# PriUVBio/optiland_Pr

Measured on AMD Instinct MI355X. Metric: ray-surface intersections/sec at 1M pupil rays, 10-surf double-Gauss, higher is better.
Workload: dtype f64

## Files before the change

include/optiland_host.h:

```cpp
#ifndef OPTILAND_HOST_H
#define OPTILAND_HOST_H

#include "optiland_rt.h"

#ifdef __cplusplus
extern "C" {
#endif

#define ORT_HOST_ABI_VERSION 3

int ort_host_abi_version(void);

int ort_host_trace_sequential(const ort_lens* lens, const ort_rays* rays_in,
                              ort_rays* rays_out, const ort_batch* batch,
                              const ort_options* opt, double* rec, int32_t* updates,
                              int32_t* status);

int ort_host_trace_sequential_vjp(const ort_lens* lens, const ort_rays* rays_in,
                                  const ort_batch* batch, const ort_options* opt,
                                  const ort_vjp_params* params, const ort_rays* cotangent,
                                  const double* rec_cotangent, const double* rec,
                                  double* grad, const ort_rays* grad_in);

int ort_host_trace_pupil(const ort_lens* lens, const double* px, const double* py,
                         ort_rays* rays_out, const ort_batch* batch, const ort_options* opt,
                         int32_t* updates, int32_t* status);

int ort_host_trace_pupil_vjp(const ort_lens* lens, const double* px, const double* py,
                             const ort_batch* batch, const ort_options* opt,
                             const ort_vjp_params* params, const ort_rays* cotangent,
                             double* grad);

int ort_host_rms_spot(const double* x, const double* y, int64_t n, double* stats, double* rms);
int ort_host_rms_spot_vjp(const double* x, const double* y, int64_t n, const double* stats,
                          const double* grad_out, double* gx, double* gy);

int ort_host_huygens_psf(const double* ix, const double* iy, const double* iz, int64_t n_image,
                         const double* px, const double* py, const double* pz,
                         const double* amp, const double* opd_mm, int64_t n_pupil,
                         double wavelength_mm, double rp, double* psf);

int ort_host_irradiance_bin(const double* x, const double* y, const double* power, int64_t n,
                            const double* x_edges, int64_t nx, const double* y_edges,
                            int64_t ny, int32_t mode, double pixel_area, double* out);
int ort_host_irradiance_bin_vjp(const double* x, const double* y, const double* power,
                                int64_t n, const double* x_edges, int64_t nx,
                                const double* y_edges, int64_t ny, double pixel_area,
                                const double* grad_out, double* grad_x, double* grad_y,
                                double* grad_power);

int ort_host_trace_pupil_polarized(const ort_lens* lens, const double* px, const double* py,
                                   ort_rays* rays_out, const ort_batch* batch,
                                   const ort_options* opt, double* rec, int32_t* updates,
                                   int32_t* status, const ort_polarization* pol);
int ort_host_trace_sequential_polarized(const ort_lens* lens, const ort_rays* rays_in,
                                        ort_rays* rays_out, const ort_batch* batch,
                                        const ort_options* opt, double* rec, int32_t* updates,
                                        int32_t* status, const ort_polarization* pol);

int ort_host_generate_rays(const double* px, const double* py, ort_rays* rays_out,
                           const ort_batch* batch);

void ort_host_set_threads(int32_t n);

#ifdef __cplusplus
}
#endif
#endif
```

include/optiland_rt.h:

```cpp
#ifndef OPTILAND_RT_H
#define OPTILAND_RT_H

#include <stdint.h>

#ifdef __cplusplus
extern "C" {
#endif

#define ORT_ABI_VERSION 21
#define ORT_MAX_SURFACES 64

enum ort_geometry {
  ORT_GEOM_PLANE = 0,
  ORT_GEOM_STANDARD = 1,
  ORT_GEOM_EVEN_ASPHERE = 2,
  ORT_GEOM_ODD_ASPHERE = 3,
  ORT_GEOM_ZERNIKE = 4,
  ORT_GEOM_POLYNOMIAL = 5,
  ORT_GEOM_CHEBYSHEV = 6,
  ORT_GEOM_BICONIC = 7,
  ORT_GEOM_TOROIDAL = 8,
  ORT_GEOM_FORBES_QBFS = 9,
  ORT_GEOM_FORBES_Q2D = 10,
  ORT_GEOM_GRID_SAG = 11,
  ORT_GEOM_NURBS = 12
};

enum ort_surface_flags {
  ORT_SURF_REFLECTIVE = 1u << 0,
  ORT_SURF_RADIUS_INF = 1u << 1,
  ORT_SURF_APERTURE = 1u << 2,
  ORT_SURF_RECORD = 1u << 3,
  ORT_SURF_TRANSLATE = 1u << 4,
  ORT_SURF_APERTURE_PROG = 1u << 5,
  ORT_SURF_INV_R2 = 1u << 6,
  ORT_SURF_ALPHA_ALL = 1u << 7,
  ORT_SURF_ALPHA_NONE = 1u << 8,
  ORT_SURF_SLOPE_INEXACT = 1u << 9
};

enum ort_lens_flags {
  ORT_LENS_AXIAL = 1u << 0
};

enum ort_interaction {
  ORT_IA_REFRACT_REFLECT = 0,
  ORT_IA_THIN_LENS = 1,
  ORT_IA_PHASE = 2,
  ORT_IA_DIFFRACTIVE = 3
};
enum ort_phase_kind { ORT_PHASE_CONSTANT = 0, ORT_PHASE_LINEAR = 1, ORT_PHASE_RADIAL = 2 };

enum ort_cs_kind {
  ORT_CS_TRANSLATE = 0,
  ORT_CS_ROT_X = 1,
  ORT_CS_ROT_Y = 2,
  ORT_CS_ROT_Z = 3
};

typedef struct ort_cs_op {
  int32_t kind;
  int32_t reserved;
  double p[3];
} ort_cs_op;

typedef struct ort_surface {
  double radius;
  double conic;
  double tol;
  double norm_radius;
  double ap_rmax2;
  double ap_rmin2;
  int32_t geometry;
  int32_t flags;
  int32_t max_iter;
  int32_t n_coef;
  int32_t coef_off;
  int32_t mat_pre;
  int32_t mat_post;
  int32_t cs_loc_off;
  int32_t n_cs_loc;
  int32_t cs_glob_off;
  int32_t n_cs_glob;
  int32_t rec_slot;
  double cs_t[3];
  int32_t ap_off;
  int32_t ap_len;
  int32_t interaction;
  int32_t ia_off;
  double inv_r2;
  double two_r;
  double one_plus_k;
  double r_sq;
  int32_t zm_off;
  int32_t zm_deg;
} ort_surface;

enum ort_aperture_op {
  ORT_AP_RADIAL = 1,
  ORT_AP_ELLIPSE = 2,
  ORT_AP_RECT = 3,
  ORT_AP_POLYGON = 4,
  ORT_AP_UNION = 5,
  ORT_AP_INTERSECT = 6,
  ORT_AP_DIFFERENCE = 7
};

typedef struct ort_surface_optics {
  double n_pre;
  double u;
  double alpha_pre;
  double n_post;
  double u_sq;
} ort_surface_optics;

typedef struct ort_zernike_term {
  double c;
  double norm;
  int32_t n;
  int32_t m;
  int32_t rad_off;
  int32_t n_rad;
} ort_zernike_term;

enum ort_material_kind {
  ORT_MAT_IDEAL = 0,
  ORT_MAT_FORMULA_1 = 1,
  ORT_MAT_TABULATED = 10,
  ORT_MAT_ABBE = 11
};
typedef struct ort_material {
  int32_t kind;
  int32_t n_coef;
  int32_t coef_off;
  int32_t k_len;
  int32_t k_off;
  int32_t reserved;
  double n_const;
  double k_const;
} ort_material;

typedef struct ort_lens {
  const ort_surface* surfaces;
  const ort_cs_op* cs_ops;
  const double* coef;
  const ort_zernike_term* zern;
  const double* n_tab;
  const double* alpha_tab;
  const ort_surface_optics* optics;
  int32_t n_surfaces;
  int32_t n_lambda;
  int32_t n_mat;
  int32_t final_mat;
  uint32_t geometry_mask;
  uint32_t interaction_mask;
  double final_thickness;
  const ort_material* materials;
  const double* wavelengths;
  uint32_t frame_flags;
  uint32_t reserved;
} ort_lens;

typedef struct ort_rays {
  double* x;
  double* y;
  double* z;
  double* L;
  double* M;
  double* N;
  double* i;
  double* opd;
} ort_rays;

enum ort_gen_mode {
  ORT_GEN_INFINITE = 0,
  ORT_GEN_FINITE = 1,
  ORT_GEN_TELECENTRIC = 2
};
typedef struct ort_segment {
  double epd;
  double epl;
  double vx, vy;
  double x_off;
  double y_off;
  double z0;
  int32_t lambda_idx;
  int32_t mode;
} ort_segment;

enum ort_apod_kind {
  ORT_APOD_UNIFORM = 0,
  ORT_APOD_GAUSSIAN = 1,
  ORT_APOD_COSINE_SQUARED = 2,
  ORT_APOD_HANN = 3,
  ORT_APOD_POLYNOMIAL = 4,
// ... 297 lines not shown
```

optiland_pr_amd/_abi.py:

```python

from __future__ import annotations

import numpy as np

ABI_VERSION = 21
HUYGENS_CHUNK = 512
BIN_HISTOGRAM = 0
BIN_BILINEAR = 1
IRRADIANCE_TILE_PIXELS = 16384
IRRADIANCE_MAX_PIXELS = 1 << 26
VJP_UNROLLED = 0
VJP_ADJOINT = 1
AP_RADIAL = 1
AP_ELLIPSE = 2
AP_RECT = 3
AP_POLYGON = 4
AP_UNION = 5
AP_INTERSECT = 6
AP_DIFFERENCE = 7
PUPIL_UNIFORM = 0
PUPIL_HEXAPOLAR = 1
PUPIL_RANDOM = 2
PUPIL_RING = 3
PUPIL_LINE_X = 4
PUPIL_LINE_Y = 5
PUPIL_CROSS = 6
MAX_SURFACES = 64

GEOM_PLANE = 0
GEOM_STANDARD = 1
GEOM_EVEN_ASPHERE = 2
GEOM_ODD_ASPHERE = 3
GEOM_ZERNIKE = 4
GEOM_POLYNOMIAL = 5
GEOM_CHEBYSHEV = 6
GEOM_BICONIC = 7
GEOM_TOROIDAL = 8
GEOM_FORBES_QBFS = 9
GEOM_FORBES_Q2D = 10
GEOM_GRID_SAG = 11
GEOM_NURBS = 12
FREEFORM_GEOMETRIES = (GEOM_POLYNOMIAL, GEOM_CHEBYSHEV, GEOM_BICONIC, GEOM_TOROIDAL,
                       GEOM_FORBES_QBFS, GEOM_FORBES_Q2D, GEOM_GRID_SAG)
NEWTON_GEOMETRIES = (GEOM_EVEN_ASPHERE, GEOM_ODD_ASPHERE, GEOM_ZERNIKE) + FREEFORM_GEOMETRIES

SURF_REFLECTIVE = 1 << 0
SURF_RADIUS_INF = 1 << 1
SURF_APERTURE = 1 << 2
SURF_RECORD = 1 << 3
SURF_TRANSLATE = 1 << 4
SURF_APERTURE_PROG = 1 << 5
SURF_INV_R2 = 1 << 6
SURF_ALPHA_ALL = 1 << 7
SURF_ALPHA_NONE = 1 << 8
SURF_SLOPE_INEXACT = 1 << 9
LENS_AXIAL = 1 << 0

IA_REFRACT_REFLECT = 0
IA_THIN_LENS = 1
IA_PHASE = 2
IA_DIFFRACTIVE = 3
PHASE_CONSTANT = 0
PHASE_LINEAR = 1
PHASE_RADIAL = 2

CS_TRANSLATE = 0
CS_ROT_X = 1
CS_ROT_Y = 2
CS_ROT_Z = 3

GEN_INFINITE = 0
GEN_FINITE = 1
GEN_TELECENTRIC = 2

APOD_UNIFORM = 0
APOD_GAUSSIAN = 1
APOD_COSINE_SQUARED = 2
APOD_HANN = 3
APOD_POLYNOMIAL = 4
APOD_SUPER_GAUSSIAN = 5
APOD_TUKEY = 6

NEWTON_SCHEDULE = 0
NEWTON_WAVE = 1

STATUS_ZERNIKE_RANGE = 1 << 0
STATUS_CHEBYSHEV_RANGE = 1 << 1
STATUS_BAD_GEOMETRY = 1 << 2
STATUS_BAD_APODIZATION = 1 << 3

CS_OP = np.dtype(
    [("kind", "<i4"), ("reserved", "<i4"), ("p", "<f8", (3,))], align=True
)
assert CS_OP.itemsize == 32

SURFACE = np.dtype(
    [
        ("radius", "<f8"),
        ("conic", "<f8"),
        ("tol", "<f8"),
        ("norm_radius", "<f8"),
        ("ap_rmax2", "<f8"),
        ("ap_rmin2", "<f8"),
        ("geometry", "<i4"),
        ("flags", "<i4"),
        ("max_iter", "<i4"),
        ("n_coef", "<i4"),
        ("coef_off", "<i4"),
        ("mat_pre", "<i4"),
        ("mat_post", "<i4"),
        ("cs_loc_off", "<i4"),
        ("n_cs_loc", "<i4"),
        ("cs_glob_off", "<i4"),
        ("n_cs_glob", "<i4"),
        ("rec_slot", "<i4"),
        ("cs_t", "<f8", (3,)),
        ("ap_off", "<i4"),
        ("ap_len", "<i4"),
        ("interaction", "<i4"),
        ("ia_off", "<i4"),
        ("inv_r2", "<f8"),
        ("two_r", "<f8"),
        ("one_plus_k", "<f8"),
        ("r_sq", "<f8"),
        ("zm_off", "<i4"),
        ("zm_deg", "<i4"),
    ],
    align=True,
)
assert SURFACE.itemsize == 176

SURFACE_OPTICS = np.dtype(
    [("n_pre", "<f8"), ("u", "<f8"), ("alpha_pre", "<f8"), ("n_post", "<f8"), ("u_sq", "<f8")],
    align=True,
)
assert SURFACE_OPTICS.itemsize == 40

ZERNIKE_TERM = np.dtype(
    [
        ("c", "<f8"),
        ("norm", "<f8"),
        ("n", "<i4"),
        ("m", "<i4"),
        ("rad_off", "<i4"),
        ("n_rad", "<i4"),
    ],
    align=True,
)
assert ZERNIKE_TERM.itemsize == 32

SEGMENT = np.dtype(
    [
        ("epd", "<f8"),
        ("epl", "<f8"),
        ("vx", "<f8"),
        ("vy", "<f8"),
        ("x_off", "<f8"),
        ("y_off", "<f8"),
        ("z0", "<f8"),
        ("lambda_idx", "<i4"),
        ("mode", "<i4"),
    ],
    align=True,
)
assert SEGMENT.itemsize == 64

APODIZATION = np.dtype(
    [
        ("kind", "<i4"),
        ("reserved", "<i4"),
        ("p", "<f8", (4,)),
    ],
    align=True,
)
assert APODIZATION.itemsize == 40

COAT_NONE = 0
COAT_SIMPLE = 1
COAT_FRESNEL = 2
COATING = np.dtype(
    [
        ("kind", "<i4"),
        ("mat_pre", "<i4"),
        ("mat_post", "<i4"),
        ("reserved", "<i4"),
        ("transmittance", "<f8"),
        ("reflectance", "<f8"),
    ],
    align=True,
)
assert COATING.itemsize == 32
POL_IGNORE = 0
POL_MATRICES = 1
POL_POLARIZED = 2
POL_UNPOLARIZED = 3

MAT_IDEAL = 0
MAT_TABULATED = 10
MAT_ABBE = 11

MATERIAL = np.dtype(
    [
        ("kind", "<i4"),
        ("n_coef", "<i4"),
        ("coef_off", "<i4"),
        ("k_len", "<i4"),
        ("k_off", "<i4"),
        ("reserved", "<i4"),
        ("n_const", "<f8"),
# ... 30 lines not shown
```

optiland_pr_amd/csrc/ort_args.h:

```cpp
#pragma once

#include "ort_core.h"
#include "ort_interact.h"
#include "ort_material.h"
#include "ort_polar.h"

namespace ortk {

#if defined(__HIP_DEVICE_COMPILE__)
#define ORT_CONST_AS __attribute__((address_space(4)))
#else
#define ORT_CONST_AS
#endif
template <class T>
using cptr = const ORT_CONST_AS T*;
template <class T>
ORT_INLINE cptr<T> cst(const T* p) {
  return (cptr<T>)(p);
}
using PD = cptr<double>;
using PZ = cptr<ort_zernike_term>;
constexpr ort::ZSeed kNoSeed{nullptr, 0};

enum : uint32_t {
  F_KM = 15u | ort::KM_NURBS,
  F_GEN = 1u << 4,
  F_REC = 1u << 5,
  F_MONO = 1u << 6,
  F_WRAY = 1u << 7,
  F_IA = 1u << 8,
  F_AXIAL = 1u << 9,
  F_TAPE = 1u << 10,
  F_SPOT = 1u << 11,
  F_RMS = 1u << 12,
  F_STRIDE = 1u << 13,
  F_POL = 1u << 14,
};
constexpr uint32_t kAllKinds =
    ort::KM_EVEN | ort::KM_ODD | ort::KM_ZERN | ort::KM_FREE | ort::KM_NURBS;

constexpr int kTapeRows = 11;
constexpr int kHist = 4;

ORT_INLINE int tape_rows(const ort_surface& s) {
  return (s.geometry == ORT_GEOM_PLANE || s.geometry == ORT_GEOM_STANDARD) ? 7 : kTapeRows;
}
ORT_INLINE int64_t tape_row0(const ort_surface* surf, int si) {
  int64_t r = 0;
  for (int k = 0; k < si; ++k) r += tape_rows(cst(surf)[k]);
  return r;
}

struct KArgs {
  const ort_surface* surf;
  const ort_cs_op* cs;
  const double* coef;
  const ort_zernike_term* zern;
  const double* n_tab;
  const double* alpha_tab;
  const ort_surface_optics* optics;
  int32_t n_surf;
  int32_t n_lambda;
  int32_t n_mat;
  int32_t final_mat;
  double final_thickness;
  ort_rays in;
  ort_rays out;
  const double* px;
  const double* py;
  int64_t n_rays;
  int64_t seg_len;
  int64_t group_len;
  const ort_segment* seg;
  int32_t n_seg;
  int32_t pupil_per_ray;
  int32_t newton_mode;
  int32_t start_surface;
  const int32_t* sched;
  int32_t conv_base;
  double* rec;
  ort_newton_stat* stats;
  int32_t* status;
  const double* w;
  const ort_material* mats;
  const double* lambdas;
  const ort_apodization* apod;
  int32_t block_remap;
  const int32_t* run_if;
  int32_t no_init;
  int32_t exact_only;
  const ort_newton_stat* vstats;
  const int32_t* vprev;
  int32_t* vflag;
  int32_t* sched_out;
  double* tape;
  double* spot_part1;
  const ort_cs_op* spot_ops;
  int32_t spot_n_ops;
  int32_t spot_chunks;
  double* rms_part;
  const ort_coating* coat;
  int32_t pol_mode;
  ort::Cplx pol_ex, pol_ey;
  double* p_out;
};

inline int fill_pol(KArgs& a, const ort_batch* batch, const ort_options* opt,
                    const ort_polarization* pol, uint32_t& feat) {
  if (!pol || !pol->coatings || batch->w || opt->tape || opt->rms_part) return ORT_ERR_ARG;
  if (pol->mode < ORT_POL_IGNORE || pol->mode > ORT_POL_UNPOLARIZED) return ORT_ERR_ARG;
  if (feat & (F_IA | F_WRAY | ort::KM_NURBS)) return ORT_ERR_ARG;
  a.coat = pol->coatings;
  a.pol_mode = pol->mode;
  a.pol_ex = {pol->ex_re, pol->ex_im};
  a.pol_ey = {pol->ey_re, pol->ey_im};
  a.p_out = pol->p_out;
  feat |= F_POL;
  return ORT_OK;
}

inline int fill_args(KArgs& a, const ort_lens* lens, const ort_batch* batch,
                     const ort_options* opt, double* rec, ort_newton_stat* stats,
                     int32_t* status, uint32_t& feat) {
  if (!lens || !batch || !opt) return ORT_ERR_ARG;
  if (lens->n_surfaces < 0 || lens->n_surfaces > ORT_MAX_SURFACES) return ORT_ERR_SURFACES;
  if (lens->n_surfaces > 0 &&
      (!lens->surfaces || !lens->n_tab || !lens->alpha_tab || !lens->optics))
    return ORT_ERR_ARG;
  if (batch->n_rays < 0 || batch->seg_len < 1 || batch->group_len < 1) return ORT_ERR_ARG;
  if (lens->n_lambda < 1 || lens->n_mat < 1) return ORT_ERR_ARG;
  if (opt->start_surface < 0) return ORT_ERR_ARG;
  a.surf = lens->surfaces;
  a.cs = lens->cs_ops;
  a.coef = lens->coef;
  a.zern = lens->zern;
  a.n_tab = lens->n_tab;
  a.alpha_tab = lens->alpha_tab;
  a.optics = lens->optics;
  a.n_surf = lens->n_surfaces;
  a.n_lambda = lens->n_lambda;
  a.n_mat = lens->n_mat;
  a.final_mat = lens->final_mat;
  a.final_thickness = lens->final_thickness;
  a.n_rays = batch->n_rays;
  a.seg_len = batch->seg_len;
  a.group_len = batch->group_len;
  a.seg = batch->seg;
  a.n_seg = batch->n_seg;
  a.pupil_per_ray = batch->pupil_per_ray;
  a.apod = batch->apod;
  a.newton_mode = opt->newton_mode;
  a.start_surface = opt->start_surface;
  a.sched = opt->sched;
  a.conv_base = opt->conv_base;
  a.run_if = opt->run_if;
  a.no_init = (opt->flags & ORT_OPT_NO_INIT) != 0;
  a.exact_only = (opt->flags & ORT_OPT_EXACT) != 0;
  a.tape = opt->tape;
  a.rms_part = opt->rms_part;
  if (opt->conv_base < 0) return ORT_ERR_ARG;
  if (lens->geometry_mask & ~((2u << ORT_GEOM_NURBS) - 1u)) return ORT_ERR_ARG;
  a.rec = rec;
  a.stats = stats;
  a.status = status;
  feat = 0;
  if (lens->geometry_mask & (1u << ORT_GEOM_EVEN_ASPHERE)) feat |= ort::KM_EVEN;
  if (lens->geometry_mask & (1u << ORT_GEOM_ODD_ASPHERE)) feat |= ort::KM_ODD;
  if (lens->geometry_mask & (1u << ORT_GEOM_ZERNIKE)) feat |= ort::KM_ZERN;
  if (lens->geometry_mask & ((1u << ORT_GEOM_POLYNOMIAL) | (1u << ORT_GEOM_CHEBYSHEV) |
                             (1u << ORT_GEOM_BICONIC) | (1u << ORT_GEOM_TOROIDAL) |
                             (1u << ORT_GEOM_FORBES_QBFS) | (1u << ORT_GEOM_FORBES_Q2D) |
                             (1u << ORT_GEOM_GRID_SAG)))
    feat |= ort::KM_FREE;
  if (lens->geometry_mask & (1u << ORT_GEOM_NURBS))
    feat |= ort::KM_NURBS | F_IA | ort::KM_EVEN | ort::KM_ODD | ort::KM_ZERN | ort::KM_FREE;
  if (rec) feat |= F_REC;
  if (batch->w) {
    if (!lens->materials) return ORT_ERR_ARG;
    a.w = batch->w;
    a.mats = lens->materials;
    feat |= F_WRAY;
  } else if (lens->n_lambda == 1 || batch->n_seg <= 1 || batch->seg_len % 64 == 0) {
    feat |= F_MONO;
  }
  if (lens->interaction_mask & ~(1u << ORT_IA_REFRACT_REFLECT)) {
    feat |= F_IA;
    a.lambdas = lens->wavelengths;
    const uint32_t need_w = (1u << ORT_IA_PHASE) | (1u << ORT_IA_DIFFRACTIVE);
    if ((lens->interaction_mask & need_w) && !batch->w && !lens->wavelengths) return ORT_ERR_ARG;
  }
  if (lens->frame_flags & ORT_LENS_AXIAL) feat |= F_AXIAL;
  if (opt->newton_mode != ORT_NEWTON_SCHEDULE && opt->newton_mode != ORT_NEWTON_WAVE)
    return ORT_ERR_ARG;
  a.vstats = opt->verify_stats;
  a.vprev = opt->verify_prev_flag;
  a.vflag = opt->verify_flag;
  a.sched_out = opt->sched_out;
  if (opt->verify_stats) {
    const int64_t ng = (batch->n_rays + batch->group_len - 1) / batch->group_len;
    if ((feat & F_KM) == 0 || opt->newton_mode != ORT_NEWTON_SCHEDULE || !opt->sched ||
        !opt->verify_flag || !opt->sched_out || opt->sched_out == opt->sched ||
        !(opt->flags & ORT_OPT_NO_INIT) ||
        opt->run_if || ng * (int64_t)lens->n_surfaces > ORT_VERIFY_MAX_SCHED)
      return ORT_ERR_ARG;
  }
  return ORT_OK;
}

ORT_INLINE double tab(const double* t, int n_lambda, int n_mat, int lam, int mat) {
  if (n_lambda == 1) return cst(t)[mat];
  return t[lam * n_mat + mat];
}

ORT_INLINE ort_surface_optics optics_row(const KArgs& a, int lam, int si) {
  if (a.n_lambda == 1) return cst(a.optics)[si];
  return a.optics[lam * a.n_surf + si];
}

ORT_INLINE ort_surface_optics optics_ray(const KArgs& a, const ort_surface& s, double w) {
  const ort_material mp = cst(a.mats)[s.mat_pre];
  const ort_material mq = cst(a.mats)[s.mat_post];
  ort_surface_optics o;
  o.n_pre = ort::material_n(mp, a.coef, w);
  o.n_post = ort::material_n(mq, a.coef, w);
  o.u = o.n_pre / o.n_post;
  o.u_sq = o.u * o.u;
  o.alpha_pre = ort::absorption_alpha(ort::material_k(mp, a.coef, w), w);
  return o;
}

template <class T>
ORT_INLINE void localize(const KArgs& a, const ort_surface& s, ort::RayT<T>& r) {
  {
    r.x = r.x + -s.cs_t[0];
    r.y = r.y + -s.cs_t[1];
  }
  r.z = r.z + -s.cs_t[2];
  for (int c = 0; c < s.n_cs_loc; ++c) ort::apply_cs_op(r, cst(a.cs)[s.cs_loc_off + c]);
}

template <class T>
ORT_INLINE void globalize(const KArgs& a, const ort_surface& s, ort::RayT<T>& r) {
  for (int c = 0; c < s.n_cs_glob; ++c) ort::apply_cs_op(r, cst(a.cs)[s.cs_glob_off + c]);
  r.x = r.x + s.cs_t[0];
  r.y = r.y + s.cs_t[1];
  r.z = r.z + s.cs_t[2];
}

ORT_INLINE bool known_geometry(int g) { return g >= ORT_GEOM_PLANE && g <= ORT_GEOM_NURBS; }
ORT_INLINE bool scheduled_geometry(int g) {
  return g != ORT_GEOM_PLANE && g != ORT_GEOM_STANDARD && g != ORT_GEOM_NURBS;
}

ORT_INLINE int range_bit(const ort_surface& s) {
  return s.geometry == ORT_GEOM_CHEBYSHEV ? (int)ORT_STATUS_CHEBYSHEV_RANGE
                                          : (int)ORT_STATUS_ZERNIKE_RANGE;
}

template <uint32_t KM, bool WRAY>
ORT_INLINE void interact(const KArgs& a, const ort_surface& s, ort::Ray& r,
                         const ort_surface_optics& o, int lam, double wl, bool& unnorm) {
  const bool refl = (s.flags & ORT_SURF_REFLECTIVE) != 0;
  const PD p = cst(a.coef) + s.ia_off;
  if (s.interaction == ORT_IA_THIN_LENS) {
    ort::thin_lens(r, p[0], o.n_pre, refl ? -o.n_pre : o.n_post);
    unnorm = true;
    return;
  }
  double nx, ny, nz;
  ort::surface_normal<KM>(s, s.radius, s.conic, cst(a.coef), cst(a.zern), kNoSeed, r, nx, ny,
                          nz);
  if (s.interaction == ORT_IA_REFRACT_REFLECT) {
    if (refl)
      ort::reflect(r, nx, ny, nz);
    else
      ort::refract(r, nx, ny, nz, o.u);
    return;
  }
  double w = wl;
  if constexpr (!WRAY) w = a.n_lambda == 1 ? cst(a.lambdas)[0] : a.lambdas[lam];
  if (s.interaction == ORT_IA_PHASE)
    ort::phase_interact(r, p, nx, ny, nz, o.n_pre, refl ? o.n_pre : o.n_post, refl, w);
  else
    ort::diffract(r, p, nx, ny, nz, o.n_pre, o.n_post, refl, w);
}

template <uint32_t KM>
ORT_INLINE void pol_step(const KArgs& a, const ort_surface& s, const ort_surface_optics& o,
                         int si, int lam, ort::Ray& r, ort::PolState& pol, bool hn,
                         double& nx, double& ny, double& nz) {
  if (!hn)
    ort::surface_normal<KM>(s, s.radius, s.conic, cst(a.coef), cst(a.zern), kNoSeed, r, nx, ny,
                            nz);
  const double k0x = r.L, k0y = r.M, k0z = r.N;
  const bool refl = (s.flags & ORT_SURF_REFLECTIVE) != 0;
  if (refl)
    ort::reflect(r, nx, ny, nz);
  else
    ort::refract(r, nx, ny, nz, o.u);
  const ort_coating ct = cst(a.coat)[si];
  double n1 = 1.0, n2 = 1.0;
  if (ct.kind == ORT_COAT_FRESNEL) {
    n1 = tab(a.n_tab, a.n_lambda, a.n_mat, lam, ct.mat_pre);
    n2 = tab(a.n_tab, a.n_lambda, a.n_mat, lam, ct.mat_post);
  }
  ort::pol_surface(pol, ct, refl, nx, ny, nz, k0x, k0y, k0z, r.L, r.M, r.N, n1, n2, r.i);
}

ORT_INLINE void load_ray(const KArgs& a, int64_t r_ld, ort::Ray& r) {
  r.x = a.in.x[r_ld];
  r.y = a.in.y[r_ld];
  r.z = a.in.z[r_ld];
  r.L = a.in.L[r_ld];
  r.M = a.in.M[r_ld];
  r.N = a.in.N[r_ld];
  r.i = a.in.i[r_ld];
  r.opd = a.in.opd[r_ld];
  r.att = 0.0;
}

struct PlainStore {
  static ORT_INLINE void put(double& lhs, double v) { lhs = v; }
};

template <class St>
ORT_INLINE void store_ray(const KArgs& a, int64_t rid, const ort::Ray& r,
                          const double* inten = nullptr) {
  St::put(a.out.x[rid], r.x);
  St::put(a.out.y[rid], r.y);
  St::put(a.out.z[rid], r.z);
  St::put(a.out.L[rid], r.L);
  St::put(a.out.M[rid], r.M);
  St::put(a.out.N[rid], r.N);
  St::put(a.out.i[rid], inten ? *inten : ort::intensity(r));
  St::put(a.out.opd[rid], r.opd);
}

template <class St>
ORT_INLINE void store_record(const KArgs& a, const ort_surface& s, int64_t rid,
                             const ort::Ray& r, const double* apod = nullptr) {
  double* base = a.rec + (int64_t)s.rec_slot * 8 * a.n_rays + rid;
  St::put(base[0 * a.n_rays], r.x);
  St::put(base[1 * a.n_rays], r.y);
  St::put(base[2 * a.n_rays], r.z);
// ... 204 lines not shown
```

optiland_pr_amd/csrc/ort_k_closed.hip:

```cpp

#include "ort_reduce.h"

namespace ortk {
__global__ __launch_bounds__(kBlock) void generate_kernel(const KArgs a) {
  const int64_t rid = (int64_t)blockIdx.x * kBlock + threadIdx.x;
  if (rid >= a.n_rays) return;
  const int64_t sidx = rid / a.seg_len;
  const ort_segment sg = a.seg[sidx];
  const int64_t p = a.pupil_per_ray ? rid : (rid - sidx * a.seg_len);
  const ort::Ray r = ort::generate_ray(sg, a.px[p], a.py[p], a.apod);
  a.out.x[rid] = r.x;
  a.out.y[rid] = r.y;
  a.out.z[rid] = r.z;
  a.out.L[rid] = r.L;
  a.out.M[rid] = r.M;
  a.out.N[rid] = r.N;
  a.out.i[rid] = r.i;
  a.out.opd[rid] = r.opd;
}

KernelFn select_generate() { return generate_kernel; }

__global__ __launch_bounds__(kBlock) void material_nk_kernel(const ort_material* mats,
                                                             const double* coef, int32_t mat,
                                                             const double* w, int64_t n,
                                                             double* n_out, double* k_out) {
  const int64_t i = (int64_t)blockIdx.x * kBlock + threadIdx.x;
  if (i >= n) return;
  const ort_material m = mats[mat];
  const double wi = w[i];
  if (n_out) n_out[i] = ort::material_n(m, coef, wi);
  if (k_out) k_out[i] = ort::material_k(m, coef, wi);
}

void launch_material_nk(const ort_material* mats, const double* coef, int32_t mat,
                        const double* w, int64_t n, double* n_out, double* k_out,
                        hipStream_t stream) {
  const int64_t blocks = (n + kBlock - 1) / kBlock;
  hipLaunchKernelGGL(material_nk_kernel, dim3((unsigned)blocks), dim3(kBlock), 0, stream,
                     mats, coef, mat, w, n, n_out, k_out);
}

int closed_block() { return kClosedBlock; }

KernelFn select_closed(uint32_t feat) {
#ifdef ORT_NO_AXIAL
  feat &= ~F_AXIAL;
#endif
  switch (feat & (F_GEN | F_REC | F_MONO | F_WRAY | F_AXIAL | F_SPOT)) {
#define ORT_C(F) \
  case (F):      \
    return trace_closed_kernel<(F)>;        \
  case (F) | F_AXIAL:                       \
    return trace_closed_kernel<(F) | F_AXIAL>;
    ORT_C(0) ORT_C(F_GEN) ORT_C(F_REC) ORT_C(F_GEN | F_REC)
    ORT_C(F_MONO) ORT_C(F_MONO | F_GEN) ORT_C(F_MONO | F_REC) ORT_C(F_MONO | F_GEN | F_REC)
    ORT_C(F_WRAY) ORT_C(F_WRAY | F_REC)
    ORT_C(F_GEN | F_SPOT) ORT_C(F_MONO | F_GEN | F_SPOT)
#undef ORT_C
    default: return nullptr;
  }
}

}
```

optiland_pr_amd/csrc/ort_kernels.h:

```cpp

#pragma once

#include <hip/hip_runtime.h>
#include <stdlib.h>

#include "ort_args.h"
#include "ort_core.h"
#include "ort_fastpath.h"
#include "ort_interact.h"
#include "ort_material.h"

namespace ortk {

#ifndef ORT_TEMPORAL_STORE
#define ORT_ST(lhs, v) __builtin_nontemporal_store((v), &(lhs))
#else
#define ORT_ST(lhs, v) ((lhs) = (v))
#endif
struct StreamStore {
  static __device__ inline __attribute__((always_inline)) void put(double& lhs, double v) {
    ORT_ST(lhs, v);
  }
};

// ... 653 lines not shown
                                  hnx, hny, hnz, active ? tp : nullptr, sched, unused);
      } else {
        t = __builtin_nan("");
      }
    }
    if constexpr ((FEAT & F_TAPE) != 0) {
      if (active) ORT_ST(tp[6 * a.n_rays], t);
    }
    const double n_pre = o.n_pre, u = o.u, alpha = o.alpha_pre;
    if constexpr ((FEAT & F_IA) != 0) {
      ort::propagate(r, t, alpha);
      if (unnorm) {
        ort::normalize_dir(r);
        unnorm = false;
      }
      ort::add_opd(r, t, n_pre);
      if (s.flags & ORT_SURF_APERTURE) ort::clip_radial(r, s.ap_rmax2, s.ap_rmin2);
      if (s.flags & ORT_SURF_APERTURE_PROG) ort::clip_program(r, cst(a.coef) + s.ap_off, s.ap_len);
      interact<(FEAT & F_KM), (FEAT & F_WRAY) != 0>(a, s, r, o, lam, wl, unnorm);
    } else if constexpr ((FEAT & F_POL) != 0) {
      to_intersection(a, s, r, t, alpha, n_pre);
      double nx = hnx, ny = hny, nz = hnz;
      pol_step<(FEAT & F_KM)>(a, s, o, si, lam, r, pol, hn, nx, ny, nz);
    } else if constexpr ((FEAT & F_KM) != 0) {
      if (hn) {
        to_intersection(a, s, r, t, alpha, n_pre);
        if (s.flags & ORT_SURF_REFLECTIVE)
          ort::reflect(r, hnx, hny, hnz);
        else
          ort::refract(r, hnx, hny, hnz, u);
      } else {
        ort::finish_surface<(FEAT & F_KM)>(r, s, s.radius, s.conic, cst(a.coef), cst(a.zern), kNoSeed, t, n_pre, u,
                                           alpha);
      }
    } else {
      to_intersection<kApProg>(a, s, r, t, alpha, n_pre);
      double nx, ny, nz;
      if (s.geometry == ORT_GEOM_PLANE) {
        nx = 0.0; ny = 0.0; nz = 1.0;
      } else if (s.flags & ORT_SURF_INV_R2) {
        ort::normal_conic_rcp(r.x, r.y, s.radius, s.conic, s.inv_r2, nx, ny, nz);
      } else {
        ort::normal_conic(r.x, r.y, s.radius, s.conic, nx, ny, nz);
      }
      if (s.flags & ORT_SURF_REFLECTIVE)
        ort::reflect(r, nx, ny, nz);
      else
        ort::refract(r, nx, ny, nz, u);
    }
    globalize(a, s, r);
    if constexpr ((FEAT & F_REC) != 0) {
      if ((s.flags & ORT_SURF_RECORD) && active) store_record<StreamStore>(a, s, rid, r);
    }
  }
  if (a.final_mat >= 0) {
    ort::propagate(r, a.final_thickness, final_alpha<FEAT>(a, lam, wl));
    if constexpr ((FEAT & F_IA) != 0) {
      if (unnorm) ort::normalize_dir(r);
    }
  }

  if (range_bits && active && a.status) atomicOr(a.status, range_bits);
  if constexpr ((FEAT & F_RMS) != 0) rms_epilogue(a, r, active, vb);
  if (!active) return;
  if constexpr ((FEAT & F_POL) != 0) {
    const double inten = ort::pol_intensity(pol, a.pol_mode, a.pol_ex, a.pol_ey, ort::intensity(r));
    store_ray<StreamStore>(a, rid, r, &inten);
    if (a.p_out) {
#pragma unroll
      for (int e = 0; e < 9; ++e) {
        ORT_ST(a.p_out[(int64_t)(2 * e) * a.n_rays + rid], pol.re[e]);
        ORT_ST(a.p_out[(int64_t)(2 * e + 1) * a.n_rays + rid], pol.im[e]);
      }
    }
    return;
  }
  store_ray<StreamStore>(a, rid, r);
}

template <uint32_t FEAT>
__global__ __launch_bounds__(kBlock) ORT_TRACE_OCC void trace_kernel(const KArgs a) {
  if (a.run_if && *cst(a.run_if) != 1) return;
  const int32_t* sched = a.sched;
  __shared__ int32_t vsched[ORT_VERIFY_MAX_SCHED];
  __shared__ int32_t vcodes[kBlock / 64];
  if constexpr ((FEAT & F_KM) != 0) {
    if (a.vstats) {
      const int64_t ng = (a.n_rays + a.group_len - 1) / a.group_len;
      const int nsch = (int)ng * a.n_surf;
      constexpr int kPre = ORT_VERIFY_MAX_SCHED / kBlock;
      int32_t pre[kPre];
#pragma unroll
      for (int q = 0; q < kPre; ++q) {
        const int k = threadIdx.x + q * kBlock;
        pre[q] = k < nsch ? a.sched[k] : 0;
      }
      const int prev = a.vprev ? *a.vprev : 1;
      if (prev != 1) {
        if (blockIdx.x == 0) {
#pragma unroll
          for (int q = 0; q < kPre; ++q) {
            const int k = threadIdx.x + q * kBlock;
            if (k < nsch) a.sched_out[k] = pre[q];
          }
          if (threadIdx.x == 0) *a.vflag = prev;
        }
        return;
      }
#pragma unroll
      for (int q = 0; q < kPre; ++q) {
        const int k = threadIdx.x + q * kBlock;
        if (k < nsch) vsched[k] = pre[q];
      }
      __syncthreads();
      const int c = newton_decide(a.surf, a.n_surf, ng, a.vstats, a.conv_base, vsched, vcodes);
      if (blockIdx.x == 0) {
        for (int k = threadIdx.x; k < nsch; k += kBlock) a.sched_out[k] = vsched[k];
        if (threadIdx.x == 0) *a.vflag = c;
      }
      if (c != 1) return;
      sched = vsched;
    }
  }
  const int64_t nb = (a.n_rays + kBlock - 1) / kBlock;
  if constexpr ((FEAT & F_STRIDE) != 0) {
    for (int64_t vb = blockIdx.x; vb < nb; vb += gridDim.x) trace_block<FEAT>(a, sched, vb, nb);
  } else {
    trace_block<FEAT>(a, sched, blockIdx.x, nb);
  }
}

template <uint32_t FEAT, bool FAST, class B>
__device__ inline ort::Ray closed_ray_in(const KArgs& a, int64_t r_ld, int& lam, double& wl,
                                         B& bad) {
  ort::Ray r;
  if constexpr ((FEAT & F_GEN) != 0) {
    const int64_t sidx = a.n_seg == 1 ? 0 : r_ld / a.seg_len;
    const ort_segment sg = a.n_seg == 1 ? cst(a.seg)[0] : a.seg[sidx];
    lam = sg.lambda_idx;
    const int64_t p = a.pupil_per_ray ? r_ld : (r_ld - sidx * a.seg_len);
    if constexpr (FAST)
      r = ort::fast::generate_ray(sg, a.px[p], a.py[p], nullptr, bad);
    else
      r = ort::generate_ray(sg, a.px[p], a.py[p], nullptr);
  } else {
    if (a.seg) lam = a.seg[a.n_seg == 1 ? 0 : r_ld / a.seg_len].lambda_idx;
    if constexpr ((FEAT & F_WRAY) != 0) wl = a.w[r_ld];
    load_ray(a, r_ld, r);
    if constexpr (FAST) ORT_CHK(bad, !(::fabs(r.L) < __builtin_inf() && ::fabs(r.M) < __builtin_inf()));
  }
  return r;
}

template <uint32_t FEAT, bool FAST, class B>
__device__ inline void closed_surfaces(const KArgs& a, ort::Ray& r, int lam, double wl,
                                       int64_t rid, bool active, B& bad, bool& geom_bad,
                                       double apod = 1.0) {
  for (int si = a.start_surface; si < a.n_surf; ++si) {
    const ort_surface s = cst(a.surf)[si];
    const ort_surface_optics o = surface_optics<FEAT>(a, s, lam, si, wl);
    if constexpr ((FEAT & F_AXIAL) != 0)
      r.z = r.z + -s.cs_t[2];
    else
      localize(a, s, r);
    const bool is_plane = s.geometry == ORT_GEOM_PLANE;
    const bool radius_inf = (s.flags & ORT_SURF_RADIUS_INF) != 0;
    bool sbad = false;
    double t;
    if constexpr (FAST) {
      t = is_plane ? ort::fast::distance_plane(r, sbad)
                   : ort::fast::distance_conic_folded(r, s, radius_inf, sbad);
    } else {
      t = is_plane ? ort::distance_plane(r) : ort::distance_conic(r, s.radius, s.conic, radius_inf);
    }
    if constexpr (FAST) {
      ORT_CHK_UNIFORM(bad, s.geometry > ORT_GEOM_STANDARD || s.geometry < ORT_GEOM_PLANE);
    } else if (!is_plane && s.geometry != ORT_GEOM_STANDARD) {
      t = __builtin_nan("");
      geom_bad = true;
    }
#ifndef ORT_NO_ALPHA_FLAGS
    if constexpr ((FEAT & F_WRAY) != 0)
      ort::propagate(r, t, o.alpha_pre);
    else
      ort::propagate_flagged(r, t, o.alpha_pre, s.flags);
#else
    ort::propagate(r, t, o.alpha_pre);
#endif
    ort::add_opd(r, t, o.n_pre);
    if (s.flags & ORT_SURF_APERTURE) ort::clip_radial(r, s.ap_rmax2, s.ap_rmin2);
#ifndef ORT_NO_AP_PROG
    if (s.flags & ORT_SURF_APERTURE_PROG) ort::clip_program(r, cst(a.coef) + s.ap_off, s.ap_len);
#endif
    const bool refl = (s.flags & ORT_SURF_REFLECTIVE) != 0;
#ifndef ORT_NO_FLAT_FAST
    constexpr bool kFlat = FAST;
#else
    constexpr bool kFlat = false;
#endif
    if (kFlat && !refl && (is_plane || radius_inf)) {
      ort::fast::refract_flat(r, o.u, o.u_sq, sbad);
    } else {
      double nx, ny, nz;
      if (is_plane) {
        nx = 0.0; ny = 0.0; nz = 1.0;
      } else if (s.flags & ORT_SURF_INV_R2) {
        if constexpr (FAST)
          ort::fast::normal_conic_rcp(r.x, r.y, s, nx, ny, nz, sbad);
        else
          ort::normal_conic_rcp(r.x, r.y, s.radius, s.conic, s.inv_r2, nx, ny, nz);
      } else {
        ort::normal_conic(r.x, r.y, s.radius, s.conic, nx, ny, nz);
      }
      if (refl) {
        ort::reflect(r, nx, ny, nz);
      } else {
        if constexpr (FAST)
          ort::fast::refract(r, nx, ny, nz, o.u, o.u_sq, sbad);
        else
          ort::refract(r, nx, ny, nz, o.u);
      }
    }
    if constexpr ((FEAT & F_AXIAL) != 0) {
      if (!FAST || si == a.start_surface) {
        if constexpr (FAST) asm volatile("");
        r.x = r.x + 0.0;
        r.y = r.y + 0.0;
      }
      r.z = r.z + s.cs_t[2];
    } else {
      globalize(a, s, r);
    }
    if constexpr (FAST) ORT_CHK(bad, sbad);
    if constexpr ((FEAT & F_REC) != 0) {
      if ((s.flags & ORT_SURF_RECORD) && active) {
        if constexpr ((FEAT & F_GEN) != 0)
          store_record<StreamStore>(a, s, rid, r, a.apod ? &apod : nullptr);
        else
          store_record<StreamStore>(a, s, rid, r);
      }
    }
  }
}

__device__ inline const KArgs& kernarg_again() {
  auto p = (const __attribute__((address_space(4))) KArgs*)__builtin_amdgcn_kernarg_segment_ptr();
  asm volatile("" : "+s"(p));
  return (const KArgs&)*p;
}

template <uint32_t FEAT>
__global__ __launch_bounds__(kClosedBlock) __attribute__((amdgpu_waves_per_eu(8))) void trace_closed_kernel(const KArgs a0) {
  const KArgs& a = a0;
  int64_t rid;
  bool active;
  if constexpr ((FEAT & F_SPOT) != 0) {
    const int64_t pair = blockIdx.x / a.spot_chunks;
    const int64_t j = (int64_t)(blockIdx.x - pair * a.spot_chunks) * kClosedBlock + threadIdx.x;
    rid = pair * a.seg_len + j;
    active = j < a.seg_len && rid < a.n_rays;
  } else {
    rid = (int64_t)blockIdx.x * kClosedBlock + threadIdx.x;
    active = rid < a.n_rays;
  }
  const int64_t r_ld = active ? rid : 0;
  int lam = 0;
  double wl = 0.0;
  bool bad = false, geom_bad = false;
  double apod_f = 1.0;
  if constexpr ((FEAT & F_GEN) != 0 && (FEAT & F_REC) != 0) {
    if (a.apod) {
      const int64_t sidx = a.n_seg == 1 ? 0 : r_ld / a.seg_len;
      const int64_t p = a.pupil_per_ray ? r_ld : (r_ld - sidx * a.seg_len);
      apod_f = ort::apodize(*cst(a.apod), a.px[p], a.py[p]);
    }
  }
#ifndef ORT_NO_DEFERRED_CHECKS
  ort::fast::WaveFlag fbad{0};
  ort::Ray r = closed_ray_in<FEAT, true>(a, r_ld, lam, wl, fbad);
  closed_surfaces<FEAT, true>(a, r, lam, wl, rid, active, fbad, geom_bad, apod_f);
  const KArgs& b = kernarg_again();
  bad = ((fbad.m >> (threadIdx.x & 63)) & 1) != 0 || !ort::fast::state_ok(r) ||
        b.exact_only != 0;
  if (__builtin_expect(bad, 0)) {
    r = closed_ray_in<FEAT, false>(b, r_ld, lam, wl, bad);
    closed_surfaces<FEAT, false>(b, r, lam, wl, rid, active, bad, geom_bad, apod_f);
  }
#else
  const KArgs& b = a;
  ort::Ray r = closed_ray_in<FEAT, false>(b, r_ld, lam, wl, bad);
  closed_surfaces<FEAT, false>(b, r, lam, wl, rid, active, bad, geom_bad, apod_f);
#endif
  if (b.final_mat >= 0) ort::propagate(r, b.final_thickness, final_alpha<FEAT>(b, lam, wl));
  if (geom_bad && b.status && threadIdx.x == 0) atomicOr(b.status, (int)ORT_STATUS_BAD_GEOMETRY);
  if constexpr ((FEAT & F_GEN) != 0) {
    if (b.apod && b.status && threadIdx.x == 0 &&
        (uint32_t)cst(b.apod)->kind > (uint32_t)ORT_APOD_TUKEY)
      atomicOr(b.status, (int)ORT_STATUS_BAD_APODIZATION);
  }
  double inten = ort::intensity(r);
#ifndef ORT_NO_APOD
  if constexpr ((FEAT & F_GEN) != 0) {
    if (b.apod) {
      const int64_t sidx = b.n_seg == 1 ? 0 : r_ld / b.seg_len;
      const int64_t p = b.pupil_per_ray ? r_ld : (r_ld - sidx * b.seg_len);
      inten = ort::apodize(*cst(b.apod), b.px[p], b.py[p]) * inten;
    }
  }
#endif
  if constexpr ((FEAT & F_SPOT) != 0) spot_epilogue<FEAT>(b, r, inten, active);
  if (!active) return;
  store_ray<StreamStore>(b, rid, r, &inten);
}

template <int CTRL, int ROW_MASK>
__device__ inline double dpp_step(double v) {
  const long long b = __double_as_longlong(v);
  const int lo = __builtin_amdgcn_update_dpp(0, (int)(b & 0xffffffffll), CTRL, ROW_MASK, 0xf,
                                             false);
  const int hi = __builtin_amdgcn_update_dpp(0, (int)(b >> 32), CTRL, ROW_MASK, 0xf, false);
  return __longlong_as_double(((long long)hi << 32) | (long long)(unsigned)lo);
}
__device__ inline double wave_sum(double v) {
  if (__builtin_amdgcn_read_exec() == ~0ull) {
    v += dpp_step<0xB1, 0xf>(v);
    v += dpp_step<0x4E, 0xf>(v);
    v += dpp_step<0x141, 0xf>(v);
    v += dpp_step<0x140, 0xf>(v);
    v += dpp_step<0x142, 0xa>(v);
    v += dpp_step<0x143, 0xc>(v);
    const long long b = __double_as_longlong(v);
    const int lo = __builtin_amdgcn_readlane((int)(b & 0xffffffffll), 63);
    const int hi = __builtin_amdgcn_readlane((int)(b >> 32), 63);
    return __longlong_as_double(((long long)hi << 32) | (long long)(unsigned)lo);
  }
  for (int o = 32; o > 0; o >>= 1) v += __shfl_xor(v, o, 64);
  return v;
}

struct GArgs {
  int32_t surface;
  int32_t mode;
  const double* x;
  const double* y;
  double* sag;
  double* nx;
  double* ny;
  double* nz;
  double* t;
};

template <uint32_t KM>
__global__ __launch_bounds__(kBlock) void geom_kernel(const KArgs a, const GArgs g) {
  const int64_t rid = (int64_t)blockIdx.x * kBlock + threadIdx.x;
  const bool active = rid < a.n_rays;
  const int64_t r_ld = active ? rid : 0;
  const ort_surface s = cst(a.surf)[g.surface];
  bool range_error = false;
  int range_bits = 0;
// ... 79 lines not shown
```

optiland_pr_amd/lowering.py:

```python

from __future__ import annotations

from dataclasses import dataclass, field

import numpy as np

from . import _abi
from .apertures import RadialAperture, program_depth
from .geometries import (NewtonRaphsonGeometry, ZernikePolynomialGeometry, scalar,
                         zernike_monomial_block)
from .surfaces import ObjectSurface


@dataclass
class LensTable:
    surfaces: np.ndarray
    cs_ops: np.ndarray
    coef: np.ndarray
    zern: np.ndarray
    n_tab: np.ndarray
    alpha_tab: np.ndarray
    wavelengths: list
    final_mat: int
    final_thickness: float
    materials: list = field(default_factory=list)
    mat_table: np.ndarray = None
    n_rec: int = 0
    rec_surfaces: list = field(default_factory=list)
    device_coeffs: list = field(default_factory=list)
    apod: np.ndarray = None
    coatings: np.ndarray = None

    @property
    def n_surfaces(self):
        return int(self.surfaces.shape[0])

    @property
    def u_tab(self):
        pre = self.n_tab[:, self.surfaces["mat_pre"]]
        post = self.n_tab[:, self.surfaces["mat_post"]]
        return np.ascontiguousarray(pre / post)

    @property
    def optics(self):
        o = np.zeros((self.n_tab.shape[0], self.n_surfaces), dtype=_abi.SURFACE_OPTICS)
        o["n_pre"] = self.n_tab[:, self.surfaces["mat_pre"]]
        o["u"] = self.u_tab
        o["alpha_pre"] = self.alpha_tab[:, self.surfaces["mat_pre"]]
        o["n_post"] = self.n_tab[:, self.surfaces["mat_post"]]
        o["u_sq"] = o["u"] * o["u"]
        return o

    @property
    def frame_flags(self):
        s = self.surfaces
        t = s["cs_t"][:, :2]
        axial = (np.all(s["n_cs_loc"] == 0) and np.all(s["n_cs_glob"] == 0)
                 and np.all(t == 0.0) and not np.any(np.signbit(t)))
        return _abi.LENS_AXIAL if axial else 0

    @property
    def interaction_mask(self):
        m = 0
        for v in np.unique(self.surfaces["interaction"]):
            m |= 1 << int(v)
        return m

    @property
    def newton_surfaces(self):
        return [i for i, s in enumerate(self.surfaces)
                if int(s["geometry"]) in _abi.NEWTON_GEOMETRIES]

    @property
    def has_zernike(self):
        return bool(np.any(self.surfaces["geometry"] == _abi.GEOM_ZERNIKE))

    @property
    def has_range_check(self):
        g = self.surfaces["geometry"]
        return bool(np.any((g == _abi.GEOM_ZERNIKE) | (g == _abi.GEOM_CHEBYSHEV)))

    def fingerprint(self):
        parts = [np.ascontiguousarray(a).tobytes() for a in
                 (self.surfaces, self.cs_ops, self.coef, self.zern, self.n_tab, self.alpha_tab,
                  self.mat_table)]
        parts.append(np.array([self.final_mat], dtype=np.int64).tobytes())
        parts.append(np.array([self.final_thickness], dtype=np.float64).tobytes())
        if self.apod is not None:
            parts.append(np.ascontiguousarray(self.apod).tobytes())
        if self.coatings is not None and np.any(self.coatings["kind"] != _abi.COAT_NONE):
            parts.append(np.ascontiguousarray(self.coatings).tobytes())
        return b"".join(parts)


def lower_apodization(optic):
    apod = getattr(optic, "apodization", None)
    return None if apod is None else apod.lower()


def _device_tensor(v):
    return hasattr(v, "is_cuda") and bool(v.is_cuda)


_MAT_LOWER: dict = {}
_MAT_N_ALPHA: dict = {}


def _cacheable(key):
    return not (isinstance(key, tuple) and key[:1] == ("ref",))


def _material_lower(m):
    key = m.key()
    if not _cacheable(key):
        return m.lower()
    hit = _MAT_LOWER.get(key)
    if hit is None:
        if len(_MAT_LOWER) > 4096:
            _MAT_LOWER.clear()
        hit = _MAT_LOWER[key] = m.lower()
    return hit


def _material_n_alpha(m, w):
    key = (m.key(), w)
    hit = _MAT_N_ALPHA.get(key) if _cacheable(key[0]) else None
    if hit is None:
        if len(_MAT_N_ALPHA) > 65536:
            _MAT_N_ALPHA.clear()
        kv = m.k_scalar(w)
        hit = (m.n_scalar(w), (4 * np.pi * np.float64(kv) / np.float64(w)) if kv > 0 else 0.0)
        if _cacheable(key[0]):
            _MAT_N_ALPHA[key] = hit
    return hit


def lower_surface_group(surface_group, wavelengths, record=False, skip_object=True,
                        polarized=False):
    surfs = [s for s in surface_group.surfaces if not isinstance(s, ObjectSurface)]
    if len(surfs) > _abi.MAX_SURFACES:
        raise ValueError(f"at most {_abi.MAX_SURFACES} surfaces are supported")
    wavelengths = [float(w) for w in np.atleast_1d(wavelengths)]

    mats, mat_index = [], {}

    def mat_id(m):
        key = m.key()
        if key not in mat_index:
            mat_index[key] = len(mats)
            mats.append(m)
        return mat_index[key]

    if record is True:
        rec_set = list(range(len(surfs)))
    elif record:
        rec_set = sorted(int(i) for i in record)
    else:
        rec_set = []

    rows = [{} for _ in surfs]
    ops, coef, zern = [], [], []
    ap_progs = []
    ia_blocks = []
    coat_rows = []
    device_coeffs = []
    for si, s in enumerate(surfs):
        g = s.geometry
        R, k, tol, max_iter, norm_radius, cc = g.lower_params()
        row = rows[si]
        row["zm_deg"] = -1
        row["geometry"] = g.geometry_id
        row["radius"] = R
        row["conic"] = k
        row["tol"] = tol
        row["max_iter"] = max_iter
        row["norm_radius"] = norm_radius
        row["two_r"] = np.float64(2.0) * np.float64(R)
        row["one_plus_k"] = np.float64(1.0) + np.float64(k)
        row["r_sq"] = np.float64(R) * np.float64(R)
        flags = 0
        if s.is_reflective:
            flags |= _abi.SURF_REFLECTIVE
        if isinstance(g, NewtonRaphsonGeometry) or g.geometry_id == _abi.GEOM_STANDARD:
            if np.isinf(R):
                flags |= _abi.SURF_RADIUS_INF
        if g.geometry_id == _abi.GEOM_STANDARD:
            rr = np.float64(R) * np.float64(R)
            if np.isfinite(rr) and 2.0**-300 <= rr <= 2.0**300:
                row["inv_r2"] = np.float64(1.0) / rr
                flags |= _abi.SURF_INV_R2
        if s.aperture is not None:
            if type(s.aperture) is RadialAperture:
                flags |= _abi.SURF_APERTURE
                row["ap_rmax2"] = s.aperture.r_max**2
                row["ap_rmin2"] = s.aperture.r_min**2
            else:
                prog = [float(v) for v in s.aperture.program()]
                if program_depth(prog) > 32:
                    raise ValueError("aperture expression nests too deeply (32 levels)")
                flags |= _abi.SURF_APERTURE_PROG
                ap_progs.append((si, prog))
        if si in rec_set:
            flags |= _abi.SURF_RECORD
            row["rec_slot"] = rec_set.index(si)
        else:
            row["rec_slot"] = -1
        row["flags"] = flags
        if isinstance(g, ZernikePolynomialGeometry):
            on_device = _device_tensor(g.coefficients)
            terms = g.zernike_terms(values=not on_device)
            if on_device:
                device_coeffs.append((len(zern), g.coefficients))
# ... 248 lines not shown
```

Before: 193.3 billion.

## Add plain-lens kernel specialization loading only needed surface fields

Adds a LENS_PLAIN flag, computed during lowering, for lenses made only of plane/standard conic surfaces with no apertures, reflection or recording. A new F_PLAIN kernel variant for axial generated traces loads just the fields it uses rather than the whole surface and optics structs, and drops the geometry check, aperture clipping and reflect branches. The aim is to cut per-surface constant loads and branching in the closed-form trace loop, at the cost of two more kernel instantiations and a flag the lowering must set correctly.

```diff
diff --git a/include/optiland_host.h b/include/optiland_host.h
--- a/include/optiland_host.h
+++ b/include/optiland_host.h
@@ -10,6 +10,7 @@
 #define ORT_HOST_ABI_VERSION 3
 
 int ort_host_abi_version(void);
+
 
 int ort_host_trace_sequential(const ort_lens* lens, const ort_rays* rays_in,
                               ort_rays* rays_out, const ort_batch* batch,
diff --git a/include/optiland_rt.h b/include/optiland_rt.h
--- a/include/optiland_rt.h
+++ b/include/optiland_rt.h
@@ -40,7 +40,8 @@
 };
 
 enum ort_lens_flags {
-  ORT_LENS_AXIAL = 1u << 0
+  ORT_LENS_AXIAL = 1u << 0,
+  ORT_LENS_PLAIN = 1u << 1
 };
 
 enum ort_interaction {
diff --git a/optiland_pr_amd/_abi.py b/optiland_pr_amd/_abi.py
--- a/optiland_pr_amd/_abi.py
+++ b/optiland_pr_amd/_abi.py
@@ -55,6 +55,7 @@
 SURF_ALPHA_NONE = 1 << 8
 SURF_SLOPE_INEXACT = 1 << 9
 LENS_AXIAL = 1 << 0
+LENS_PLAIN = 1 << 1
 
 IA_REFRACT_REFLECT = 0
 IA_THIN_LENS = 1
diff --git a/optiland_pr_amd/csrc/ort_args.h b/optiland_pr_amd/csrc/ort_args.h
--- a/optiland_pr_amd/csrc/ort_args.h
+++ b/optiland_pr_amd/csrc/ort_args.h
@@ -35,6 +35,7 @@
   F_RMS = 1u << 12,
   F_STRIDE = 1u << 13,
   F_POL = 1u << 14,
+  F_PLAIN = 1u << 15,
 };
 constexpr uint32_t kAllKinds =
     ort::KM_EVEN | ort::KM_ODD | ort::KM_ZERN | ort::KM_FREE | ort::KM_NURBS;
@@ -190,6 +191,7 @@
     if ((lens->interaction_mask & need_w) && !batch->w && !lens->wavelengths) return ORT_ERR_ARG;
   }
   if (lens->frame_flags & ORT_LENS_AXIAL) feat |= F_AXIAL;
+  if ((lens->frame_flags & ORT_LENS_PLAIN) && (feat & (F_KM | F_IA)) == 0) feat |= F_PLAIN;
   if (opt->newton_mode != ORT_NEWTON_SCHEDULE && opt->newton_mode != ORT_NEWTON_WAVE)
     return ORT_ERR_ARG;
   a.vstats = opt->verify_stats;
diff --git a/optiland_pr_amd/csrc/ort_k_closed.hip b/optiland_pr_amd/csrc/ort_k_closed.hip
--- a/optiland_pr_amd/csrc/ort_k_closed.hip
+++ b/optiland_pr_amd/csrc/ort_k_closed.hip
@@ -47,7 +47,16 @@
 #ifdef ORT_NO_AXIAL
   feat &= ~F_AXIAL;
 #endif
-  switch (feat & (F_GEN | F_REC | F_MONO | F_WRAY | F_AXIAL | F_SPOT)) {
+  const uint32_t base = feat & (F_GEN | F_REC | F_MONO | F_WRAY | F_SPOT);
+  if ((feat & F_AXIAL) == 0 || (base != F_GEN && base != (F_GEN | F_MONO))) feat &= ~F_PLAIN;
+#ifdef ORT_NO_PLAIN
+  feat &= ~F_PLAIN;
+#endif
+  switch (feat & (F_GEN | F_REC | F_MONO | F_WRAY | F_AXIAL | F_SPOT | F_PLAIN)) {
+    case F_GEN | F_AXIAL | F_PLAIN:
+      return trace_closed_kernel<F_GEN | F_AXIAL | F_PLAIN>;
+    case F_GEN | F_MONO | F_AXIAL | F_PLAIN:
+      return trace_closed_kernel<F_GEN | F_MONO | F_AXIAL | F_PLAIN>;
 #define ORT_C(F) \
   case (F):      \
     return trace_closed_kernel<(F)>;        \
diff --git a/optiland_pr_amd/csrc/ort_kernels.h b/optiland_pr_amd/csrc/ort_kernels.h
--- a/optiland_pr_amd/csrc/ort_kernels.h
+++ b/optiland_pr_amd/csrc/ort_kernels.h
@@ -829,13 +829,69 @@
   return r;
 }
 
+struct PlainSurf {
+  double radius, conic, cs_tz, inv_r2, two_r, one_plus_k, r_sq;
+  double n_pre, u, alpha_pre, u_sq;
+  int32_t geometry, flags;
+};
+template <uint32_t FEAT>
+__device__ inline PlainSurf plain_load(const KArgs& a, int row0, int si) {
+  const cptr<ort_surface> s = cst(a.surf) + si;
+  PlainSurf p{};
+  p.radius = s->radius;
+  p.conic = s->conic;
+  p.geometry = s->geometry;
+  p.flags = s->flags;
+  p.cs_tz = s->cs_t[2];
+  p.inv_r2 = s->inv_r2;
+  p.two_r = s->two_r;
+  p.one_plus_k = s->one_plus_k;
+  p.r_sq = s->r_sq;
+  if constexpr ((FEAT & F_MONO) != 0) {
+    const cptr<ort_surface_optics> o = cst(a.optics) + (row0 + si);
+    p.n_pre = o->n_pre;
+    p.u = o->u;
+    p.alpha_pre = o->alpha_pre;
+    p.u_sq = o->u_sq;
+  }
+  return p;
+}
+__device__ inline void plain_unpack(const PlainSurf& p, ort_surface& s, ort_surface_optics& o) {
+  s.radius = p.radius;
+  s.conic = p.conic;
+  s.geometry = p.geometry;
+  s.flags = p.flags;
+  s.cs_t[2] = p.cs_tz;
+  s.inv_r2 = p.inv_r2;
+  s.two_r = p.two_r;
+  s.one_plus_k = p.one_plus_k;
+  s.r_sq = p.r_sq;
+  o.n_pre = p.n_pre;
+  o.u = p.u;
+  o.alpha_pre = p.alpha_pre;
+  o.u_sq = p.u_sq;
+}
+
 template <uint32_t FEAT, bool FAST, class B>
 __device__ inline void closed_surfaces(const KArgs& a, ort::Ray& r, int lam, double wl,
                                        int64_t rid, bool active, B& bad, bool& geom_bad,
                                        double apod = 1.0) {
+  constexpr bool kPlain = FAST && (FEAT & F_PLAIN) != 0;
+  static_assert(!kPlain || (FEAT & (F_AXIAL | F_REC | F_WRAY)) == F_AXIAL,
+                "the plain form is the axial, unrecorded, table-wavelength kernels'");
+  int row0 = 0;
+  if constexpr (kPlain && (FEAT & F_MONO) != 0) row0 = uniform_row(lam) * a.n_surf;
   for (int si = a.start_surface; si < a.n_surf; ++si) {
-    const ort_surface s = cst(a.surf)[si];
-    const ort_surface_optics o = surface_optics<FEAT>(a, s, lam, si, wl);
+    ort_surface s;
+    ort_surface_optics o;
+    if constexpr (kPlain) {
+      const PlainSurf p = plain_load<FEAT>(a, row0, si);
+      plain_unpack(p, s, o);
+      if constexpr ((FEAT & F_MONO) == 0) o = optics_at<FEAT>(a, lam, si);
+    } else {
+      s = cst(a.surf)[si];
+      o = surface_optics<FEAT>(a, s, lam, si, wl);
+    }
     if constexpr ((FEAT & F_AXIAL) != 0)
       r.z = r.z + -s.cs_t[2];
     else
@@ -850,7 +906,8 @@
     } else {
       t = is_plane ? ort::distance_plane(r) : ort::distance_conic(r, s.radius, s.conic, radius_inf);
     }
-    if constexpr (FAST) {
+    if constexpr (kPlain) {
+    } else if constexpr (FAST) {
       ORT_CHK_UNIFORM(bad, s.geometry > ORT_GEOM_STANDARD || s.geometry < ORT_GEOM_PLANE);
     } else if (!is_plane && s.geometry != ORT_GEOM_STANDARD) {
       t = __builtin_nan("");
@@ -865,11 +922,13 @@
     ort::propagate(r, t, o.alpha_pre);
 #endif
     ort::add_opd(r, t, o.n_pre);
-    if (s.flags & ORT_SURF_APERTURE) ort::clip_radial(r, s.ap_rmax2, s.ap_rmin2);
+    if constexpr (!kPlain) {
+      if (s.flags & ORT_SURF_APERTURE) ort::clip_radial(r, s.ap_rmax2, s.ap_rmin2);
 #ifndef ORT_NO_AP_PROG
-    if (s.flags & ORT_SURF_APERTURE_PROG) ort::clip_program(r, cst(a.coef) + s.ap_off, s.ap_len);
-#endif
-    const bool refl = (s.flags & ORT_SURF_REFLECTIVE) != 0;
+      if (s.flags & ORT_SURF_APERTURE_PROG) ort::clip_program(r, cst(a.coef) + s.ap_off, s.ap_len);
+#endif
+    }
+    const bool refl = !kPlain && (s.flags & ORT_SURF_REFLECTIVE) != 0;
 #ifndef ORT_NO_FLAT_FAST
     constexpr bool kFlat = FAST;
 #else
@@ -881,7 +940,7 @@
       double nx, ny, nz;
       if (is_plane) {
         nx = 0.0; ny = 0.0; nz = 1.0;
-      } else if (s.flags & ORT_SURF_INV_R2) {
+      } else if (kPlain || (s.flags & ORT_SURF_INV_R2)) {
         if constexpr (FAST)
           ort::fast::normal_conic_rcp(r.x, r.y, s, nx, ny, nz, sbad);
         else
diff --git a/optiland_pr_amd/lowering.py b/optiland_pr_amd/lowering.py
--- a/optiland_pr_amd/lowering.py
+++ b/optiland_pr_amd/lowering.py
@@ -57,7 +57,13 @@
         t = s["cs_t"][:, :2]
         axial = (np.all(s["n_cs_loc"] == 0) and np.all(s["n_cs_glob"] == 0)
                  and np.all(t == 0.0) and not np.any(np.signbit(t)))
-        return _abi.LENS_AXIAL if axial else 0
+        g, f = s["geometry"], s["flags"]
+        barred = (_abi.SURF_APERTURE | _abi.SURF_APERTURE_PROG | _abi.SURF_REFLECTIVE
+                  | _abi.SURF_RECORD)
+        conic = g == _abi.GEOM_STANDARD
+        plain = (np.all((g == _abi.GEOM_PLANE) | conic) and not np.any(f & barred)
+                 and np.all((f[conic] & (_abi.SURF_INV_R2 | _abi.SURF_RADIUS_INF)) != 0))
+        return (_abi.LENS_AXIAL if axial else 0) | (_abi.LENS_PLAIN if plain else 0)
 
     @property
     def interaction_mask(self):
```

After: 198.8 billion, median of 6. +2.9%, better.
